# lingo-db/lingo-db

Hardware: AMD Instinct MI355X
Metric: tpch_sf100_geomean_ms (lower is better)
Workload: dtype int64/int128 decimal

## Files before the change

### lingo-db_amd/csrc/ldb_core.hip

```cpp
#include "ldb_internal.h"
#include "ldb_device.h"
#include "ldb_chain.h"
#include <algorithm>
#include <cstdlib>
#include <memory>

static thread_local char g_err[1024] = "";
void ldb_set_error(const char* fmt, ...) {
   va_list ap;
   va_start(ap, fmt);
   vsnprintf(g_err, sizeof(g_err), fmt, ap);
   va_end(ap);
}
extern "C" const char* ldb_gpu_last_error(void) { return g_err; }

#include <atomic>
#include <functional>
#include <mutex>
static std::mutex g_opt_mu;
static std::atomic<int64_t> g_option_epoch{0};
static std::unordered_map<std::string, int64_t> g_opts;
int64_t ldb_option(const char* name, int64_t dflt) {
   std::lock_guard<std::mutex> lock(g_opt_mu);
   auto it = g_opts.find(name);
   if (it != g_opts.end()) return it->second;
   std::string env = "LDB_";
   for (const char* c = name; *c; c++) env += (char) toupper((unsigned char) *c);
   int64_t v = dflt;
   if (const char* e = getenv(env.c_str())) v = atoll(e);
   g_opts[name] = v;
   return v;
}
extern "C" int32_t ldb_gpu_set_option(const char* name, int64_t value) {
   if (!name) LDB_FAIL(LDB_ERR_INVALID, "set_option: NULL name");
   static const char* known[] = {"jit", "jit_min_rows", "lazy_filter", "lazy_min_rows", "join_ordered", "join_chained", "gb_ordered", "gb_sorted", "zone_maps", "zone_min_rows", "gb_direct", "gb_wgs_per_cu", "gb_partition", "gb_partition_min_rows", "join_radix", "join_radix_min_rows", "join_radix_min_table_bytes", "join_radix_part_bytes", "probe_batch", "debug_check", "join_direct", "join_rank", "join_coarse", "dict_encode", "dict_min_rows", "comm_transport", "comm_timeout_ms", "desc_cache", "desc_cache_mb", "plan_replay", "scan_single_pass", "lazy_strings", "lazy_strings_min_rows", "gb_partition_wc", "join_radix_wc", "join_radix_lds", "gb_dense_out", "gb_partition_values", "join_pair32", "gb_dense_keys", "jit_async", "jit_threads", "jit_disk_cache", "join_all_match", "topk_short_select", "gb_fits64", "join_coarse_fine", "join_coarse_filtered", "compact_wide_tiles", "compact_max_words", "join_fuse_max_conjuncts", "join_coarse_finest", "jit_min_rows_like", "scan_split", "jit_share_compiles"};
   bool ok = false;
   for (const char* k : known) ok |= strcmp(k, name) == 0;
   if (!ok) LDB_FAIL(LDB_ERR_INVALID, "set_option: unknown option '%s'", name);
   std::lock_guard<std::mutex> lock(g_opt_mu);
   g_opts[name] = value;
   g_option_epoch.fetch_add(1);
   return LDB_OK;
}
extern "C" int64_t ldb_gpu_get_option(const char* name) {
   if (!name) return -1;
   std::lock_guard<std::mutex> lock(g_opt_mu);
   auto it = g_opts.find(name);
   if (it != g_opts.end()) return it->second;
   std::string env = "LDB_";
   for (const char* c = name; *c; c++) env += (char) toupper((unsigned char) *c);
   if (const char* e = getenv(env.c_str())) return atoll(e);
   return -1;
}

double ldb_host_trace_threshold() {
   static const double thr = [] {
      const char* e = getenv("LDB_HOST_TRACE");
      return e && *e ? atof(e) : -1.0;
   }();
   return thr;
}
static size_t ldb_size_class(size_t bytes) {
   if (bytes <= 256) return 256;
   const int lg = 63 - __builtin_clzll((unsigned long long) (bytes - 1));
   const size_t step = (size_t) 1 << (lg >= 3 ? lg - 3 : 0);
   return (bytes + step - 1) / step * step;
}
static void ldb_cache_release(ldb_ctx* ctx) {
   for (auto& kv : ctx->parked)
      for (void* p : kv.second) (void) hipFreeAsync(p, ctx->stream);
   ctx->parked.clear();
   ctx->cache_bytes = 0;
}
int32_t ldb_dev_alloc(ldb_ctx* ctx, void** out, size_t bytes) {
   const size_t cls = ctx->cache_on ? ldb_size_class(bytes + 16) : bytes + 16;
   if (ctx->cache_on) {
      auto it = ctx->parked.find(cls);
      if (it != ctx->parked.end() && !it->second.empty()) {
         std::pop_heap(it->second.begin(), it->second.end(), std::greater<void*>());
         *out = it->second.back();
         it->second.pop_back();
         ctx->cache_bytes -= cls;
         ctx->live[*out] = cls;
         return LDB_OK;
      }
   }
   hipError_t e;
   {
      LdbSlow slow_("hipMallocAsync", cls);
      e = hipMallocAsync(out, cls, ctx->stream);
   }
   if (e != hipSuccess && ctx->cache_bytes) {
      (void) hipGetLastError();
      ldb_cache_release(ctx);
      (void) hipStreamSynchronize(ctx->stream);
      e = hipMallocAsync(out, cls, ctx->stream);
   }
   LDB_HIP(e);
   if (ctx->cache_on) ctx->live[*out] = cls;
   return LDB_OK;
}
void ldb_dev_free(ldb_ctx* ctx, void* p) {
   if (!p) return;
   auto dref = ctx->desc_blocks.find(p);
   if (dref != ctx->desc_blocks.end()) {
      if (dref->second > 0) dref->second--;
      else {
         ctx->desc_underflows++;
         if (ldb_host_trace_threshold() >= 0) fprintf(stderr, "[ldb] descriptor %p given back twice\n", p);
      }
      return;
   }
   if (!ctx->shared.empty()) {
      auto sh = ctx->shared.find(p);
      if (sh != ctx->shared.end()) {
         if (--sh->second == 0) ctx->shared.erase(sh);
         return;
      }
   }
   auto it = ctx->live.find(p);
   if (it == ctx->live.end()) {
      LdbSlow slow_("hipFreeAsync (untracked block)");
      (void) hipFreeAsync(p, ctx->stream);
      return;
   }
   const size_t cls = it->second;
   ctx->live.erase(it);
   if (ctx->cache_bytes + cls <= ctx->cache_cap) {
      auto& heap = ctx->parked[cls];
      heap.push_back(p);
      std::push_heap(heap.begin(), heap.end(), std::greater<void*>());
      ctx->cache_bytes += cls;
   } else {
      LdbSlow slow_("hipFreeAsync (cache full)", cls);
      (void) hipFreeAsync(p, ctx->stream);
   }
}
void ldb_dev_share(ldb_ctx* ctx, void* p) {
   if (p) ctx->shared[p]++;
}
static uint64_t desc_hash(const void* p, size_t bytes) {
   const uint8_t* b = (const uint8_t*) p;
   uint64_t h = 0x9E3779B97F4A7C15ull ^ bytes;
   size_t i = 0;
   for (; i + 8 <= bytes; i += 8) {
      uint64_t w;
      memcpy(&w, b + i, 8);
      h = (h ^ w) * 0xFF51AFD7ED558CCDull;
      h ^= h >> 29;
   }
   for (; i < bytes; i++) h = (h ^ b[i]) * 0x100000001B3ull;
   return h ^ (h >> 32);
}
static void desc_cache_drop(ldb_ctx* ctx, bool force = false) {
   for (auto it = ctx->desc_cache.begin(); it != ctx->desc_cache.end();) {
      auto ref = ctx->desc_blocks.find(it->second.dev);
      if (!force && ref != ctx->desc_blocks.end() && ref->second > 0) {
         ++it;
         continue;
      }
      (void) hipFreeAsync(it->second.dev, ctx->stream);
      ctx->desc_bytes -= std::min(ctx->desc_bytes, it->second.copy.size());
      if (ref != ctx->desc_blocks.end()) ctx->desc_blocks.erase(ref);
      it = ctx->desc_cache.erase(it);
   }
   if (force) {
      ctx->desc_blocks.clear();
      ctx->desc_bytes = 0;
   }
}
int32_t ldb_h2d_small(ldb_ctx* ctx, void* dev, const void* host, size_t bytes) {
   const size_t need = (bytes + 63) & ~(size_t) 63;
   if (ctx->h_ring && need <= LDB_RING_BYTES / 8) {
      if (ctx->ring_pos + need > LDB_RING_BYTES) {
         LdbSlow slow_("staging ring wrap: hipStreamSynchronize");
         LDB_HIP(hipStreamSynchronize(ctx->stream));
         ctx->ring_pos = 0;
      }
      void* slot = ctx->h_ring + ctx->ring_pos;
      ctx->ring_pos += need;
      memcpy(slot, host, bytes);
      LDB_HIP(hipMemcpyAsync(dev, slot, bytes, hipMemcpyHostToDevice, ctx->stream));
      return LDB_OK;
   }
   LDB_HIP(hipMemcpyAsync(dev, host, bytes, hipMemcpyHostToDevice, ctx->stream));
   return LDB_OK;
}
int32_t ldb_dev_upload(ldb_ctx* ctx, const void* host, size_t bytes, void** dev_out, bool cacheable) {
// ... 1390 lines not shown
      *zmin = (uint64_t) c.zone_min;
      *zmax = (uint64_t) c.zone_max;
   }
   return LDB_OK;
}

extern "C" int64_t ldb_gpu_table_zones(ldb_ctx* ctx, const ldb_table* t, int32_t col) {
   uint64_t a = 0, b = 0;
   if (!ctx || ldb_column_zones(ctx, t, col, &a, &b) != LDB_OK) return -1;
   return a ? (t->n_rows + LDB_ZONE_ROWS - 1) >> LDB_ZONE_SHIFT : 0;
}
__global__ void k_column_sorted(DCol col, uint64_t n, unsigned int* __restrict__ unsorted) {
   bool bad = false;
   for (uint64_t i = blockIdx.x * (uint64_t) blockDim.x + threadIdx.x + 1; i < n; i += (uint64_t) gridDim.x * blockDim.x)
      bad = bad || d_load_i64(col, (uint32_t) i) < d_load_i64(col, (uint32_t) (i - 1));
   if (__ballot(bad) && (threadIdx.x & 63) == 0) atomicOr(unsorted, 1u);
}
int32_t ldb_column_sorted(ldb_ctx* ctx, const ldb_table* t, int32_t col, bool* sorted) {
   if (!t || col < 0 || (size_t) col >= t->cols.size()) LDB_FAIL(LDB_ERR_INVALID, "column_sorted: bad column %d", col);
   const ldb_column& c = t->cols[(size_t) col];
   const int ty = c.type.type;
   const bool ok = ty == LDB_T_INT8 || ty == LDB_T_INT16 || ty == LDB_T_INT32 || ty == LDB_T_INT64 || ty == LDB_T_DATE32 ||
                   (ty == LDB_T_DECIMAL128 && c.type.precision < 19);
   if (c.sorted_state < 0) {
      if (!ok || c.validity) {
         c.sorted_state = 0;
      } else if (t->n_rows < 2) {
         c.sorted_state = 1;
      } else {
         DCol dc;
         memset(&dc, 0, sizeof(dc));
         dc.values = (uint64_t) c.values;
         dc.type = ty;
         dc.width = c.width;
         dc.precision = c.type.precision;
         dc.scale = c.type.scale;
         unsigned int* d_flag = (unsigned int*) (ctx->d_scratch + 44);
         LDB_HIP(hipMemsetAsync(d_flag, 0, 8, ctx->stream));
         hipLaunchKernelGGL(k_column_sorted, dim3(ldb_grid_for(ctx, t->n_rows, 256, 8)), dim3(256), 0, ctx->stream, dc, (uint64_t) t->n_rows, d_flag);
         uint64_t f = 0;
         LDB_TRY(ldb_read_u64(ctx, d_flag, &f));
         c.sorted_state = (f & 1) ? 0 : 1;
      }
   }
   *sorted = c.sorted_state == 1;
   return LDB_OK;
}

void ldb_order_preds(DPred* preds, int32_t n) {
   std::stable_sort(preds, preds + n, [](const DPred& a, const DPred& b) { return pred_cost(a) < pred_cost(b); });
   ldb_mark_same_col(preds, n);
}

void ldb_mark_same_col(DPred* preds, int32_t n) {
   for (int32_t p = 1; p < n; p++) {
      const DCol &a = preds[p - 1].col, &b = preds[p].col;
      preds[p].same_col = a.values == b.values && a.offsets == b.offsets && a.validity == b.validity && a.rowids == b.rowids && a.type == b.type && a.width == b.width &&
                                a.precision == b.precision
                             ? 1
                             : 0;
   }
}

struct DComposeMulti {
   uint64_t n;
   const uint32_t* sel[2];
   const uint32_t* ids[12];
   uint32_t* out[12];
   int32_t n_out;
   uint8_t which[12];
};
__global__ void k_compose_multi(DComposeMulti d) {
   for (uint64_t i = blockIdx.x * (uint64_t) blockDim.x + threadIdx.x; i < d.n; i += (uint64_t) gridDim.x * blockDim.x) {
      const uint32_t s0 = d.sel[0][i];
      const uint32_t s1 = d.sel[1] ? d.sel[1][i] : 0u;
#pragma unroll
      for (int j = 0; j < 12; j++) {
         if (j >= d.n_out) break;
         const uint32_t s = d.which[j] ? s1 : s0;
         d.out[j][i] = s == LDB_NULL_ROW ? LDB_NULL_ROW : (d.ids[j] ? d.ids[j][s] : s);
      }
   }
}
int32_t ldb_compose_rowids(ldb_ctx* ctx, const uint32_t* sel0, const uint32_t* sel1, const LdbComposeJob* jobs, int n_jobs, uint64_t n) {
   if (!n || !n_jobs) return LDB_OK;
   LdbProf prof_(ctx, "k_compose_rowids");
   for (int at = 0; at < n_jobs; at += 12) {
      DComposeMulti d;
      memset(&d, 0, sizeof(d));
      d.n = n;
      d.sel[0] = sel0;
      d.sel[1] = sel1;
      d.n_out = std::min(12, n_jobs - at);
      for (int j = 0; j < d.n_out; j++) {
         d.ids[j] = jobs[at + j].ids;
         d.out[j] = jobs[at + j].out;
         d.which[j] = (uint8_t) jobs[at + j].which;
      }
      hipLaunchKernelGGL(k_compose_multi, dim3(ldb_grid_for(ctx, (int64_t) n, 256, 8)), dim3(256), 0, ctx->stream, d);
   }
   LDB_HIP(hipGetLastError());
   return LDB_OK;
}

template <typename T>
__global__ void k_gather_fixed(const T* __restrict__ src, const uint32_t* __restrict__ rowids, T* __restrict__ dst, uint64_t n) {
   for (uint64_t i = blockIdx.x * (uint64_t) blockDim.x + threadIdx.x; i < n; i += (uint64_t) gridDim.x * blockDim.x) {
      uint32_t r = rowids ? rowids[i] : (uint32_t) i;
      T v{};
      if (r != LDB_NULL_ROW) v = src[r];
      dst[i] = v;
   }
}
__global__ void k_gather_validity(const uint8_t* __restrict__ validity, const uint32_t* __restrict__ rowids, uint64_t* __restrict__ bitmap_words, uint64_t n,
                                  unsigned long long* __restrict__ null_count) {
   const uint64_t n_pad = (n + 63) & ~(uint64_t) 63;
   for (uint64_t i = blockIdx.x * (uint64_t) blockDim.x + threadIdx.x; i < n_pad; i += (uint64_t) gridDim.x * blockDim.x) {
      bool ok = false;
      if (i < n) {
         const uint32_t r = rowids ? rowids[i] : (uint32_t) i;
         ok = r != LDB_NULL_ROW && (!validity || ((validity[r >> 3] >> (r & 7)) & 1));
      }
      const uint64_t m = __ballot(ok);
      if ((threadIdx.x & 63) == 0) {
         bitmap_words[i >> 6] = m;
         const uint64_t rows_here = n - i >= 64 ? ~(uint64_t) 0 : (((uint64_t) 1 << (n - i)) - 1);
         const int nulls = __popcll(~m & rows_here);
         if (nulls) atomicAdd(null_count, (unsigned long long) nulls);
      }
   }
}
__global__ void k_str_lens(const int64_t* __restrict__ offsets, const uint32_t* __restrict__ rowids, int64_t* __restrict__ lens, uint64_t n) {
   for (uint64_t i = blockIdx.x * (uint64_t) blockDim.x + threadIdx.x; i < n; i += (uint64_t) gridDim.x * blockDim.x) {
      uint32_t r = rowids ? rowids[i] : (uint32_t) i;
      lens[i] = r == LDB_NULL_ROW ? 0 : offsets[r + 1] - offsets[r];
   }
}
__global__ void k_str_copy(const uint8_t* __restrict__ src, const int64_t* __restrict__ src_off, const uint32_t* __restrict__ rowids,
                           int64_t* __restrict__ dst_off, uint8_t* __restrict__ dst, uint64_t n, int64_t total) {
   if (blockIdx.x == 0 && threadIdx.x == 0) dst_off[n] = total;
   for (uint64_t i = blockIdx.x * (uint64_t) blockDim.x + threadIdx.x; i < n; i += (uint64_t) gridDim.x * blockDim.x) {
      uint32_t r = rowids ? rowids[i] : (uint32_t) i;
      if (r == LDB_NULL_ROW) continue;
      int64_t b = src_off[r], len = src_off[r + 1] - b, d = dst_off[i];
      if (d + len > total) len = total > d ? total - d : 0;
      for (int64_t k = 0; k < len; k++) dst[d + k] = src[b + k];
   }
}

struct u128x {
   uint64_t a, b;
};

int32_t ldb_gather_columns(ldb_ctx* ctx, const ldb_rel* r, const ldb_colref* refs, int32_t n_cols, ldb_column* outs) {
   const uint64_t n = (uint64_t) r->n_rows;
   const int grid = ldb_grid_for(ctx, (int64_t) n, 256, 8);
   struct Pending {
      int32_t col;
      int slot_nulls = -1, slot_bytes = -1;
      const uint32_t* rowids = nullptr;
      int64_t* lens = nullptr;
   };
   std::vector<Pending> pend((size_t) n_cols);
   int n_slots = 0;
   const bool lazy_on = ldb_option("lazy_strings", 1) != 0;
   const uint64_t lazy_min = (uint64_t) ldb_option("lazy_strings_min_rows", 4096);
   std::vector<ldb_column*> lazy_small;
   for (int32_t c = 0; c < n_cols; c++) {
      const ldb_rel_side& side = r->sides[(size_t) refs[c].side];
      const ldb_column& src = side.table->cols[(size_t) refs[c].col];
      pend[(size_t) c].col = c;
      if (src.validity || (side.rowids && side.may_null)) pend[(size_t) c].slot_nulls = n_slots++;
      const bool will_be_lazy = src.type.type == LDB_T_UTF8 && src.dict_codes && src.dict && (ldb_column_is_lazy(src) || (n >= 64 && n >= lazy_min && lazy_on));
      if (src.type.type == LDB_T_UTF8 && !will_be_lazy) pend[(size_t) c].slot_bytes = n_slots++;
   }
   unsigned long long* d_words = nullptr;
   if (n_slots) LDB_TRY(ldb_counters(ctx, n_slots, (uint64_t**) &d_words));
   LdbProf prof_(ctx, "k_gather");
   for (int32_t c = 0; c < n_cols; c++) {
      Pending& p = pend[(size_t) c];
      p.rowids = r->sides[(size_t) refs[c].side].rowids;
      const ldb_column& src = r->sides[(size_t) refs[c].side].table->cols[(size_t) refs[c].col];
      ldb_column* out = &outs[c];
      out->name = src.name;
      out->type = src.type;
      out->width = src.width;
      out->owned = true;
      if (p.slot_nulls >= 0) {
         LDB_TRY(ldb_dev_alloc(ctx, (void**) &out->validity, (size_t) ((n + 7) / 8 + 8)));
         if (n) hipLaunchKernelGGL(k_gather_validity, dim3(grid), dim3(256), 0, ctx->stream, src.validity, p.rowids, (uint64_t*) out->validity, n, d_words + p.slot_nulls);
      }
      const bool src_lazy = ldb_column_is_lazy(src);
      if (src.type.type == LDB_T_UTF8 && src.dict_codes && src.dict && (n >= 64 || src_lazy)) {
         LDB_TRY(ldb_dev_alloc(ctx, (void**) &out->dict_codes, 4 * (size_t) (n ? n : 1)));
         if (n) hipLaunchKernelGGL(k_gather_fixed<uint32_t>, dim3(grid), dim3(256), 0, ctx->stream, (const uint32_t*) src.dict_codes, p.rowids, out->dict_codes, n);
         out->dict = src.dict;
         out->dict->dict_refs++;
         out->dict_size = src.dict_size;
         out->dict_pred_cache = new std::unordered_map<std::string, std::string>();
      }
      if (src.type.type == LDB_T_UTF8 && out->dict_codes && (src_lazy || (n >= lazy_min && lazy_on))) {
         out->value_bytes = -1;
         p.slot_bytes = -1;
         lazy_small.push_back(src_lazy && n < 64 ? out : nullptr);
      } else if (src.type.type == LDB_T_UTF8) {
         LDB_TRY(ldb_dev_alloc(ctx, (void**) &p.lens, sizeof(int64_t) * (size_t) (n + 1)));
         LDB_TRY(ldb_dev_alloc(ctx, (void**) &out->offsets, sizeof(int64_t) * (size_t) (n + 1)));
         hipLaunchKernelGGL(k_str_lens, dim3(grid), dim3(256), 0, ctx->stream, src.offsets, p.rowids, p.lens, n);
         LDB_TRY(ldb_exclusive_scan_i64(ctx, p.lens, out->offsets, (int64_t) n, (int64_t*) (d_words + p.slot_bytes)));
      } else {
         out->value_bytes = (int64_t) n * src.width;
         if (src.has_range && p.slot_nulls < 0) {
            out->has_range = true;
            out->vmin = src.vmin;
            out->vmax = src.vmax;
         }
         LDB_TRY(ldb_dev_alloc(ctx, &out->values, (size_t) out->value_bytes));
         switch (src.width) {
            case 1: hipLaunchKernelGGL(k_gather_fixed<uint8_t>, dim3(grid), dim3(256), 0, ctx->stream, (const uint8_t*) src.values, p.rowids, (uint8_t*) out->values, n); break;
            case 2: hipLaunchKernelGGL(k_gather_fixed<uint16_t>, dim3(grid), dim3(256), 0, ctx->stream, (const uint16_t*) src.values, p.rowids, (uint16_t*) out->values, n); break;
            case 4: hipLaunchKernelGGL(k_gather_fixed<uint32_t>, dim3(grid), dim3(256), 0, ctx->stream, (const uint32_t*) src.values, p.rowids, (uint32_t*) out->values, n); break;
            case 8: hipLaunchKernelGGL(k_gather_fixed<uint64_t>, dim3(grid), dim3(256), 0, ctx->stream, (const uint64_t*) src.values, p.rowids, (uint64_t*) out->values, n); break;
            default: hipLaunchKernelGGL(k_gather_fixed<u128x>, dim3(grid), dim3(256), 0, ctx->stream, (const u128x*) src.values, p.rowids, (u128x*) out->values, n); break;
         }
      }
   }
   LDB_HIP(hipGetLastError());
   auto finish_lazy = [&]() -> int32_t {
      for (ldb_column* lc : lazy_small)
         if (lc) LDB_TRY(ldb_column_strings(ctx, *lc, (int64_t) n));
      return LDB_OK;
   };
   if (!n_slots) return finish_lazy();
   std::vector<unsigned long long> words((size_t) n_slots);
   LDB_TRY(LDB_READBACK(ctx, words.data(), d_words, 8 * (size_t) n_slots));
   for (int32_t c = 0; c < n_cols; c++) {
      Pending& p = pend[(size_t) c];
      ldb_column* out = &outs[c];
      if (p.slot_nulls >= 0) {
         out->null_count = (int64_t) words[(size_t) p.slot_nulls];
         if (out->null_count == 0) {
            ldb_dev_free(ctx, out->validity);
            out->validity = nullptr;
         }
      }
      if (p.slot_bytes >= 0) {
         const ldb_column& src = r->sides[(size_t) refs[c].side].table->cols[(size_t) refs[c].col];
         const uint64_t total = words[(size_t) p.slot_bytes];
         ldb_dev_free(ctx, p.lens);
         out->value_bytes = (int64_t) total;
         LDB_TRY(ldb_dev_alloc(ctx, &out->values, (size_t) total));
         hipLaunchKernelGGL(k_str_copy, dim3(grid), dim3(256), 0, ctx->stream, (const uint8_t*) src.values, src.offsets, p.rowids, out->offsets, (uint8_t*) out->values, n,
                            (int64_t) total);
      }
   }
   LDB_HIP(hipGetLastError());
   return finish_lazy();
}
int32_t ldb_gather_column(ldb_ctx* ctx, const ldb_rel* r, ldb_colref ref, ldb_column* out) { return ldb_gather_columns(ctx, r, &ref, 1, out); }

int32_t ldb_column_strings(ldb_ctx* ctx, const ldb_column& cc, int64_t n_rows) {
   if (!ldb_column_is_lazy(cc)) return LDB_OK;
   ldb_column& c = const_cast<ldb_column&>(cc);
   const ldb_column& dict = c.dict->cols[0];
   const uint64_t n = (uint64_t) n_rows;
   const int grid = ldb_grid_for(ctx, n_rows, 256, 8);
   int64_t *lens = nullptr, *offsets = nullptr;
   LdbBufs tmp(ctx);
   LDB_TRY(tmp.alloc(&lens, 8 * (size_t) (n + 1)));
   LDB_TRY(tmp.alloc(&offsets, 8 * (size_t) (n + 1)));
   uint64_t* d_total;
   LDB_TRY(ldb_counters(ctx, 1, &d_total));
   if (n) hipLaunchKernelGGL(k_str_lens, dim3(grid), dim3(256), 0, ctx->stream, (const int64_t*) dict.offsets, (const uint32_t*) c.dict_codes, lens, n);
   LDB_TRY(ldb_exclusive_scan_i64(ctx, lens, offsets, n_rows, (int64_t*) d_total));
   uint64_t total = 0;
   LDB_TRY(ldb_read_u64(ctx, d_total, &total));
   void* values = nullptr;
   LDB_TRY(tmp.alloc((uint8_t**) &values, (size_t) total));
   hipLaunchKernelGGL(k_str_copy, dim3(grid > 0 ? grid : 1), dim3(256), 0, ctx->stream, (const uint8_t*) dict.values, (const int64_t*) dict.offsets, (const uint32_t*) c.dict_codes, offsets, (uint8_t*) values, n,
                      (int64_t) total);
   LDB_HIP(hipGetLastError());
   tmp.keep(offsets);
   tmp.keep(values);
   c.offsets = offsets;
   c.values = values;
   c.value_bytes = (int64_t) total;
   return LDB_OK;
}

extern "C" int32_t ldb_gpu_materialize(ldb_ctx* ctx, ldb_rel* r, const ldb_colref* cols, int32_t n_cols, ldb_table** out) {
   if (!ctx || !r || !out || n_cols < 0) LDB_FAIL(LDB_ERR_INVALID, "materialize: bad argument");
   LDB_TRY(ldb_rel_force(ctx, r));
   for (int32_t c = 0; c < n_cols; c++)
      if (cols[c].side < 0 || (size_t) cols[c].side >= r->sides.size() || cols[c].col < 0 || (size_t) cols[c].col >= r->sides[(size_t) cols[c].side].table->cols.size())
         LDB_FAIL(LDB_ERR_INVALID, "materialize: column %d:%d out of range", cols[c].side, cols[c].col);
   auto t = std::make_unique<ldb_table>();
   t->ctx = ctx;
   t->name = "materialized";
   t->n_rows = r->n_rows;
   t->cols.resize((size_t) n_cols);
   int32_t s = ldb_gather_columns(ctx, r, cols, n_cols, t->cols.data());
   if (s != LDB_OK) {
      ldb_gpu_table_release(ctx, t.release());
      return s;
   }
   *out = t.release();
   return LDB_OK;
}

template <typename T, typename TO, typename TT, int VBITS>
__global__ __launch_bounds__(256) void k_scan_chain(const T* __restrict__ in, TO* __restrict__ out, uint64_t n, uint64_t n_tiles, TT* __restrict__ total,
                                                    unsigned long long* __restrict__ status, unsigned long long* __restrict__ ticket, unsigned long long ticket_base,
                                                    unsigned long long epoch) {
   __shared__ unsigned long long s_tile;
   __shared__ TO s_wave[4];
   __shared__ TO s_prefix;
   if (threadIdx.x == 0) s_tile = atomicAdd(ticket, 1ull) - ticket_base;
   __syncthreads();
   const uint64_t tile = s_tile;
   const uint64_t base = tile * CHAIN_TILE + (uint64_t) threadIdx.x * CHAIN_ITEMS;
   TO v[CHAIN_ITEMS];
   TO sum = 0;
#pragma unroll
   for (int k = 0; k < CHAIN_ITEMS; k++) {
      v[k] = base + k < n ? (TO) in[base + k] : (TO) 0;
      sum += v[k];
   }
   TO agg;
   TO excl = d_block_scan256<TO>(sum, s_wave, &agg);
   if (threadIdx.x < 64) {
      const TO prefix = d_chain_prefix<TO, VBITS>(status, tile, epoch, agg, threadIdx.x);
      if (threadIdx.x == 0) s_prefix = prefix;
   }
   __syncthreads();
   excl += s_prefix;
   if (total && tile == n_tiles - 1 && threadIdx.x == 0) *total = (TT) (s_prefix + agg);
#pragma unroll
   for (int k = 0; k < CHAIN_ITEMS; k++) {
      if (base + k < n) out[base + k] = excl;
      excl += v[k];
   }
}
int32_t ldb_chain_begin(ldb_ctx* ctx, uint64_t n_tiles, bool wide, ChainCall* c) {
   if (!ctx->scan_ticket) {
      LDB_HIP(hipMalloc((void**) &ctx->scan_ticket, 64));
      LDB_HIP(hipMemsetAsync(ctx->scan_ticket, 0, 64, ctx->stream));
      ctx->scan_ticket_base = 0;
   }
   if (n_tiles > ctx->scan_status_tiles) {
      size_t want = 4096;
      while (want < n_tiles) want *= 2;
      uint64_t* fresh = nullptr;
      LDB_HIP(hipMallocAsync((void**) &fresh, 16 * want, ctx->stream));
      LDB_HIP(hipMemsetAsync(fresh, 0, 16 * want, ctx->stream));
      if (ctx->scan_status) (void) hipFreeAsync(ctx->scan_status, ctx->stream);
      ctx->scan_status = fresh;
      ctx->scan_status_tiles = want;
   }
   ctx->scan_epoch++;
   const uint32_t mask = wide ? (1u << 20) - 1 : (1u << 30) - 1;
   if ((ctx->scan_epoch & ((1u << 20) - 1)) == 0) {
      LDB_HIP(hipMemsetAsync(ctx->scan_status, 0, 16 * ctx->scan_status_tiles, ctx->stream));
      ctx->scan_epoch++;
   }
   c->status = (unsigned long long*) ctx->scan_status + (wide ? ctx->scan_status_tiles : 0);
   c->ticket = ctx->scan_ticket;
   c->ticket_base = ctx->scan_ticket_base;
   c->epoch = ctx->scan_epoch & mask;
   ctx->scan_ticket_base += n_tiles;
   return LDB_OK;
}
int32_t ldb_chain_failed(ldb_ctx* ctx) {
   (void) hipMemsetAsync(ctx->scan_ticket, 0, 64, ctx->stream);
   ctx->scan_ticket_base = 0;
   LDB_FAIL(LDB_ERR_HIP, "chained scan: the launch failed");
}

template <typename T, typename TO, typename TT>
__global__ void k_scan_block(const T* __restrict__ in, TO* __restrict__ out, TO* __restrict__ block_sums, uint64_t n, TT* __restrict__ total) {
   __shared__ TO sh[256];
   const int ITEMS = 8;
   uint64_t base = (uint64_t) blockIdx.x * 256 * ITEMS + (uint64_t) threadIdx.x * ITEMS;
   TO v[ITEMS];
   TO sum = 0;
#pragma unroll
   for (int k = 0; k < ITEMS; k++) {
      v[k] = base + k < n ? (TO) in[base + k] : (TO) 0;
      sum += v[k];
   }
   sh[threadIdx.x] = sum;
   __syncthreads();
   for (int off = 1; off < 256; off <<= 1) {
      TO t = threadIdx.x >= (unsigned) off ? sh[threadIdx.x - off] : (TO) 0;
      __syncthreads();
      sh[threadIdx.x] += t;
      __syncthreads();
   }
   TO excl = sh[threadIdx.x] - sum;
   if (threadIdx.x == 255) {
      if (block_sums) block_sums[blockIdx.x] = sh[255];
      if (total && gridDim.x == 1) *total = (TT) sh[255];
   }
#pragma unroll
   for (int k = 0; k < ITEMS; k++) {
      if (base + k < n) out[base + k] = excl;
      excl += v[k];
   }
// ... 163 lines not shown
```

Measured before the change: 3.598.

## Batch column gathers into multi-column kernels to cut launch count

```diff
diff --git a/lingo-db_amd/csrc/ldb_core.hip b/lingo-db_amd/csrc/ldb_core.hip
--- a/lingo-db_amd/csrc/ldb_core.hip
+++ b/lingo-db_amd/csrc/ldb_core.hip
@@ -33,7 +33,7 @@
 }
 extern "C" int32_t ldb_gpu_set_option(const char* name, int64_t value) {
    if (!name) LDB_FAIL(LDB_ERR_INVALID, "set_option: NULL name");
-   static const char* known[] = {"jit", "jit_min_rows", "lazy_filter", "lazy_min_rows", "join_ordered", "join_chained", "gb_ordered", "gb_sorted", "zone_maps", "zone_min_rows", "gb_direct", "gb_wgs_per_cu", "gb_partition", "gb_partition_min_rows", "join_radix", "join_radix_min_rows", "join_radix_min_table_bytes", "join_radix_part_bytes", "probe_batch", "debug_check", "join_direct", "join_rank", "join_coarse", "dict_encode", "dict_min_rows", "comm_transport", "comm_timeout_ms", "desc_cache", "desc_cache_mb", "plan_replay", "scan_single_pass", "lazy_strings", "lazy_strings_min_rows", "gb_partition_wc", "join_radix_wc", "join_radix_lds", "gb_dense_out", "gb_partition_values", "join_pair32", "gb_dense_keys", "jit_async", "jit_threads", "jit_disk_cache", "join_all_match", "topk_short_select", "gb_fits64", "join_coarse_fine", "join_coarse_filtered", "compact_wide_tiles", "compact_max_words", "join_fuse_max_conjuncts", "join_coarse_finest", "jit_min_rows_like", "scan_split", "jit_share_compiles"};
+   static const char* known[] = {"jit", "jit_min_rows", "lazy_filter", "lazy_min_rows", "join_ordered", "join_chained", "gb_ordered", "gb_sorted", "zone_maps", "zone_min_rows", "gb_direct", "gb_wgs_per_cu", "gb_partition", "gb_partition_min_rows", "join_radix", "join_radix_min_rows", "join_radix_min_table_bytes", "join_radix_part_bytes", "probe_batch", "debug_check", "join_direct", "join_rank", "join_coarse", "dict_encode", "dict_min_rows", "comm_transport", "comm_timeout_ms", "desc_cache", "desc_cache_mb", "plan_replay", "scan_single_pass", "lazy_strings", "lazy_strings_min_rows", "gb_partition_wc", "join_radix_wc", "join_radix_lds", "gb_dense_out", "gb_partition_values", "join_pair32", "gb_dense_keys", "jit_async", "jit_threads", "jit_disk_cache", "join_all_match", "topk_short_select", "gb_fits64", "join_coarse_fine", "join_coarse_filtered", "compact_wide_tiles", "compact_max_words", "join_fuse_max_conjuncts", "join_coarse_finest", "jit_min_rows_like", "scan_split", "jit_share_compiles", "gather_multi"};
    bool ok = false;
    for (const char* k : known) ok |= strcmp(k, name) == 0;
    if (!ok) LDB_FAIL(LDB_ERR_INVALID, "set_option: unknown option '%s'", name);
@@ -1730,6 +1730,128 @@
    uint64_t a, b;
 };
 
+#define LDB_GM_JOBS 12
+#define LDB_GM_VALID 4
+struct DGatherMulti {
+   uint64_t n;
+   const uint32_t* rowids;
+   const void* src[LDB_GM_JOBS];
+   void* dst[LDB_GM_JOBS];
+   const uint8_t* vsrc[LDB_GM_VALID];
+   uint64_t* vdst[LDB_GM_VALID];
+   unsigned long long* vnulls[LDB_GM_VALID];
+   int32_t n_jobs, n_valid;
+   uint8_t width[LDB_GM_JOBS];
+};
+__global__ __launch_bounds__(256) void k_gather_multi(DGatherMulti d) {
+   const uint64_t n = d.n, n_pad = (n + 63) & ~(uint64_t) 63;
+   for (uint64_t i = blockIdx.x * (uint64_t) blockDim.x + threadIdx.x; i < n_pad; i += (uint64_t) gridDim.x * blockDim.x) {
+      const bool in = i < n;
+      uint32_t r = LDB_NULL_ROW;
+      if (in) r = d.rowids ? d.rowids[i] : (uint32_t) i;
+      const bool live = r != LDB_NULL_ROW;
+      u128x v[LDB_GM_JOBS];
+#pragma unroll
+      for (int j = 0; j < LDB_GM_JOBS; j++) {
+         v[j].a = v[j].b = 0;
+         if (j >= d.n_jobs || !live) continue;
+         switch (d.width[j]) {
+            case 1: v[j].a = ((const uint8_t*) d.src[j])[r]; break;
+            case 2: v[j].a = ((const uint16_t*) d.src[j])[r]; break;
+            case 4: v[j].a = ((const uint32_t*) d.src[j])[r]; break;
+            case 8: v[j].a = ((const uint64_t*) d.src[j])[r]; break;
+            default: v[j] = ((const u128x*) d.src[j])[r]; break;
+         }
+      }
+      bool ok[LDB_GM_VALID];
+#pragma unroll
+      for (int j = 0; j < LDB_GM_VALID; j++) ok[j] = j < d.n_valid && live && (!d.vsrc[j] || ((d.vsrc[j][r >> 3] >> (r & 7)) & 1));
+#pragma unroll
+      for (int j = 0; j < LDB_GM_JOBS; j++) {
+         if (j >= d.n_jobs || !in) continue;
+         switch (d.width[j]) {
+            case 1: ((uint8_t*) d.dst[j])[i] = (uint8_t) v[j].a; break;
+            case 2: ((uint16_t*) d.dst[j])[i] = (uint16_t) v[j].a; break;
+            case 4: ((uint32_t*) d.dst[j])[i] = (uint32_t) v[j].a; break;
+            case 8: ((uint64_t*) d.dst[j])[i] = v[j].a; break;
+            default: ((u128x*) d.dst[j])[i] = v[j]; break;
+         }
+      }
+#pragma unroll
+      for (int j = 0; j < LDB_GM_VALID; j++) {
+         if (j >= d.n_valid) break;
+         const uint64_t m = __ballot(ok[j]);
+         if ((threadIdx.x & 63) == 0) {
+            d.vdst[j][i >> 6] = m;
+            const uint64_t rows_here = n - i >= 64 ? ~(uint64_t) 0 : (((uint64_t) 1 << (n - i)) - 1);
+            const int nulls = __popcll(~m & rows_here);
+            if (nulls) atomicAdd(d.vnulls[j], (unsigned long long) nulls);
+         }
+      }
+   }
+}
+#define LDB_STR_SMALL_ROWS 2048
+#define LDB_SM_COLS 8
+struct DStrMulti {
+   uint64_t n;
+   int32_t n_cols;
+   const uint32_t* rowids[LDB_SM_COLS];
+   const int64_t* src_off[LDB_SM_COLS];
+   const uint8_t* src[LDB_SM_COLS];
+   int64_t* dst_off[LDB_SM_COLS];
+   uint8_t* dst[LDB_SM_COLS];
+   int64_t* total_out[LDB_SM_COLS];
+   int64_t total[LDB_SM_COLS];
+};
+__global__ __launch_bounds__(256) void k_str_offsets_multi(DStrMulti d) {
+   __shared__ int64_t sh[256];
+   const int c = (int) blockIdx.x;
+   const uint32_t* rowids = d.rowids[c];
+   const int64_t* off = d.src_off[c];
+   const uint64_t base = (uint64_t) threadIdx.x * 8;
+   int64_t v[8];
+   int64_t sum = 0;
+#pragma unroll
+   for (int k = 0; k < 8; k++) {
+      v[k] = 0;
+      if (base + k < d.n) {
+         const uint32_t r = rowids ? rowids[base + k] : (uint32_t) (base + k);
+         if (r != LDB_NULL_ROW) v[k] = off[r + 1] - off[r];
+      }
+      sum += v[k];
+   }
+   sh[threadIdx.x] = sum;
+   __syncthreads();
+   for (int o = 1; o < 256; o <<= 1) {
+      const int64_t t = threadIdx.x >= (unsigned) o ? sh[threadIdx.x - o] : 0;
+      __syncthreads();
+      sh[threadIdx.x] += t;
+      __syncthreads();
+   }
+   int64_t excl = sh[threadIdx.x] - sum;
+   if (threadIdx.x == 255) *d.total_out[c] = sh[255];
+#pragma unroll
+   for (int k = 0; k < 8; k++) {
+      if (base + k < d.n) d.dst_off[c][base + k] = excl;
+      excl += v[k];
+   }
+}
+__global__ __launch_bounds__(256) void k_str_copy_multi(DStrMulti d) {
+   const int c = (int) blockIdx.y;
+   const int64_t total = d.total[c];
+   int64_t* dst_off = d.dst_off[c];
+   if (blockIdx.x == 0 && threadIdx.x == 0) dst_off[d.n] = total;
+   const uint32_t* rowids = d.rowids[c];
+   for (uint64_t i = blockIdx.x * (uint64_t) blockDim.x + threadIdx.x; i < d.n; i += (uint64_t) gridDim.x * blockDim.x) {
+      const uint32_t r = rowids ? rowids[i] : (uint32_t) i;
+      if (r == LDB_NULL_ROW) continue;
+      const int64_t b = d.src_off[c][r], at = dst_off[i];
+      int64_t len = d.src_off[c][r + 1] - b;
+      if (at + len > total) len = total > at ? total - at : 0;
+      for (int64_t k = 0; k < len; k++) d.dst[c][at + k] = d.src[c][b + k];
+   }
+}
+
 int32_t ldb_gather_columns(ldb_ctx* ctx, const ldb_rel* r, const ldb_colref* refs, int32_t n_cols, ldb_column* outs) {
    const uint64_t n = (uint64_t) r->n_rows;
    const int grid = ldb_grid_for(ctx, (int64_t) n, 256, 8);
@@ -1738,6 +1860,37 @@
       int slot_nulls = -1, slot_bytes = -1;
       const uint32_t* rowids = nullptr;
       int64_t* lens = nullptr;
+      bool small_str = false;
+   };
+   const bool multi = ldb_option("gather_multi", 1) != 0;
+   struct FixedJob {
+      const uint32_t* rowids;
+      const void* src;
+      void* dst;
+      int width;
+   };
+   struct ValidJob {
+      const uint32_t* rowids;
+      const uint8_t* src;
+      uint64_t* dst;
+      unsigned long long* nulls;
+   };
+   std::vector<FixedJob> fixed_jobs;
+   std::vector<ValidJob> valid_jobs;
+   std::vector<int32_t> small_strs;
+   auto gather_fixed = [&](const void* src, const uint32_t* rowids, void* dst, int width) {
+      if (!n) return;
+      if (multi) {
+         fixed_jobs.push_back({rowids, src, dst, width});
+         return;
+      }
+      switch (width) {
+         case 1: hipLaunchKernelGGL(k_gather_fixed<uint8_t>, dim3(grid), dim3(256), 0, ctx->stream, (const uint8_t*) src, rowids, (uint8_t*) dst, n); break;
+         case 2: hipLaunchKernelGGL(k_gather_fixed<uint16_t>, dim3(grid), dim3(256), 0, ctx->stream, (const uint16_t*) src, rowids, (uint16_t*) dst, n); break;
+         case 4: hipLaunchKernelGGL(k_gather_fixed<uint32_t>, dim3(grid), dim3(256), 0, ctx->stream, (const uint32_t*) src, rowids, (uint32_t*) dst, n); break;
+         case 8: hipLaunchKernelGGL(k_gather_fixed<uint64_t>, dim3(grid), dim3(256), 0, ctx->stream, (const uint64_t*) src, rowids, (uint64_t*) dst, n); break;
+         default: hipLaunchKernelGGL(k_gather_fixed<u128x>, dim3(grid), dim3(256), 0, ctx->stream, (const u128x*) src, rowids, (u128x*) dst, n); break;
+      }
    };
    std::vector<Pending> pend((size_t) n_cols);
    int n_slots = 0;
@@ -1766,12 +1919,13 @@
       out->owned = true;
       if (p.slot_nulls >= 0) {
          LDB_TRY(ldb_dev_alloc(ctx, (void**) &out->validity, (size_t) ((n + 7) / 8 + 8)));
-         if (n) hipLaunchKernelGGL(k_gather_validity, dim3(grid), dim3(256), 0, ctx->stream, src.validity, p.rowids, (uint64_t*) out->validity, n, d_words + p.slot_nulls);
+         if (n && multi) valid_jobs.push_back({p.rowids, src.validity, (uint64_t*) out->validity, d_words + p.slot_nulls});
+         else if (n) hipLaunchKernelGGL(k_gather_validity, dim3(grid), dim3(256), 0, ctx->stream, src.validity, p.rowids, (uint64_t*) out->validity, n, d_words + p.slot_nulls);
       }
       const bool src_lazy = ldb_column_is_lazy(src);
       if (src.type.type == LDB_T_UTF8 && src.dict_codes && src.dict && (n >= 64 || src_lazy)) {
          LDB_TRY(ldb_dev_alloc(ctx, (void**) &out->dict_codes, 4 * (size_t) (n ? n : 1)));
-         if (n) hipLaunchKernelGGL(k_gather_fixed<uint32_t>, dim3(grid), dim3(256), 0, ctx->stream, (const uint32_t*) src.dict_codes, p.rowids, out->dict_codes, n);
+         gather_fixed(src.dict_codes, p.rowids, out->dict_codes, 4);
          out->dict = src.dict;
          out->dict->dict_refs++;
          out->dict_size = src.dict_size;
@@ -1781,6 +1935,10 @@
          out->value_bytes = -1;
          p.slot_bytes = -1;
          lazy_small.push_back(src_lazy && n < 64 ? out : nullptr);
+      } else if (src.type.type == LDB_T_UTF8 && multi && n <= LDB_STR_SMALL_ROWS) {
+         LDB_TRY(ldb_dev_alloc(ctx, (void**) &out->offsets, sizeof(int64_t) * (size_t) (n + 1)));
+         p.small_str = true;
+         small_strs.push_back(c);
       } else if (src.type.type == LDB_T_UTF8) {
          LDB_TRY(ldb_dev_alloc(ctx, (void**) &p.lens, sizeof(int64_t) * (size_t) (n + 1)));
          LDB_TRY(ldb_dev_alloc(ctx, (void**) &out->offsets, sizeof(int64_t) * (size_t) (n + 1)));
@@ -1794,14 +1952,53 @@
             out->vmax = src.vmax;
          }
          LDB_TRY(ldb_dev_alloc(ctx, &out->values, (size_t) out->value_bytes));
-         switch (src.width) {
-            case 1: hipLaunchKernelGGL(k_gather_fixed<uint8_t>, dim3(grid), dim3(256), 0, ctx->stream, (const uint8_t*) src.values, p.rowids, (uint8_t*) out->values, n); break;
-            case 2: hipLaunchKernelGGL(k_gather_fixed<uint16_t>, dim3(grid), dim3(256), 0, ctx->stream, (const uint16_t*) src.values, p.rowids, (uint16_t*) out->values, n); break;
-            case 4: hipLaunchKernelGGL(k_gather_fixed<uint32_t>, dim3(grid), dim3(256), 0, ctx->stream, (const uint32_t*) src.values, p.rowids, (uint32_t*) out->values, n); break;
-            case 8: hipLaunchKernelGGL(k_gather_fixed<uint64_t>, dim3(grid), dim3(256), 0, ctx->stream, (const uint64_t*) src.values, p.rowids, (uint64_t*) out->values, n); break;
-            default: hipLaunchKernelGGL(k_gather_fixed<u128x>, dim3(grid), dim3(256), 0, ctx->stream, (const u128x*) src.values, p.rowids, (u128x*) out->values, n); break;
-         }
-      }
+         gather_fixed(src.values, p.rowids, out->values, src.width);
+      }
+   }
+   for (size_t f0 = 0, v0 = 0; f0 < fixed_jobs.size() || v0 < valid_jobs.size();) {
+      const uint32_t* rowids = f0 < fixed_jobs.size() ? fixed_jobs[f0].rowids : valid_jobs[v0].rowids;
+      DGatherMulti d;
+      memset(&d, 0, sizeof(d));
+      d.n = n;
+      d.rowids = rowids;
+      auto fend = std::stable_partition(fixed_jobs.begin() + (ptrdiff_t) f0, fixed_jobs.end(), [&](const FixedJob& j) { return j.rowids == rowids; });
+      auto vend = std::stable_partition(valid_jobs.begin() + (ptrdiff_t) v0, valid_jobs.end(), [&](const ValidJob& j) { return j.rowids == rowids; });
+      const size_t nf = std::min<size_t>(LDB_GM_JOBS, (size_t) (fend - fixed_jobs.begin()) - f0), nv = std::min<size_t>(LDB_GM_VALID, (size_t) (vend - valid_jobs.begin()) - v0);
+      for (size_t j = 0; j < nf; j++) {
+         d.src[j] = fixed_jobs[f0 + j].src;
+         d.dst[j] = fixed_jobs[f0 + j].dst;
+         d.width[j] = (uint8_t) fixed_jobs[f0 + j].width;
+      }
+      for (size_t j = 0; j < nv; j++) {
+         d.vsrc[j] = valid_jobs[v0 + j].src;
+         d.vdst[j] = valid_jobs[v0 + j].dst;
+         d.vnulls[j] = valid_jobs[v0 + j].nulls;
+      }
+      d.n_jobs = (int32_t) nf;
+      d.n_valid = (int32_t) nv;
+      f0 += nf;
+      v0 += nv;
+      hipLaunchKernelGGL(k_gather_multi, dim3(grid), dim3(256), 0, ctx->stream, d);
+   }
+   auto str_desc = [&](size_t at, DStrMulti* d) {
+      memset(d, 0, sizeof(*d));
+      d->n = n;
+      d->n_cols = (int32_t) std::min<size_t>(LDB_SM_COLS, small_strs.size() - at);
+      for (int32_t j = 0; j < d->n_cols; j++) {
+         const int32_t c = small_strs[at + (size_t) j];
+         const ldb_column& src = r->sides[(size_t) refs[c].side].table->cols[(size_t) refs[c].col];
+         d->rowids[j] = pend[(size_t) c].rowids;
+         d->src_off[j] = src.offsets;
+         d->src[j] = (const uint8_t*) src.values;
+         d->dst_off[j] = outs[c].offsets;
+         d->dst[j] = (uint8_t*) outs[c].values;
+         d->total_out[j] = (int64_t*) (d_words + pend[(size_t) c].slot_bytes);
+      }
+   };
+   for (size_t at = 0; n && at < small_strs.size(); at += LDB_SM_COLS) {
+      DStrMulti d;
+      str_desc(at, &d);
+      hipLaunchKernelGGL(k_str_offsets_multi, dim3((unsigned) d.n_cols), dim3(256), 0, ctx->stream, d);
    }
    LDB_HIP(hipGetLastError());
    auto finish_lazy = [&]() -> int32_t {
@@ -1828,9 +2025,16 @@
          ldb_dev_free(ctx, p.lens);
          out->value_bytes = (int64_t) total;
          LDB_TRY(ldb_dev_alloc(ctx, &out->values, (size_t) total));
-         hipLaunchKernelGGL(k_str_copy, dim3(grid), dim3(256), 0, ctx->stream, (const uint8_t*) src.values, src.offsets, p.rowids, out->offsets, (uint8_t*) out->values, n,
+         if (!p.small_str)
+            hipLaunchKernelGGL(k_str_copy, dim3(grid), dim3(256), 0, ctx->stream, (const uint8_t*) src.values, src.offsets, p.rowids, out->offsets, (uint8_t*) out->values, n,
                             (int64_t) total);
       }
+   }
+   for (size_t at = 0; at < small_strs.size(); at += LDB_SM_COLS) {
+      DStrMulti d;
+      str_desc(at, &d);
+      for (int32_t j = 0; j < d.n_cols; j++) d.total[j] = outs[small_strs[at + (size_t) j]].value_bytes;
+      hipLaunchKernelGGL(k_str_copy_multi, dim3((unsigned) ((n + 255) / 256 ? (n + 255) / 256 : 1), (unsigned) d.n_cols), dim3(256), 0, ctx->stream, d);
    }
    LDB_HIP(hipGetLastError());
    return finish_lazy();
```

Measured after the change: 3.662. 1.8% more time.
